# yewzijian/RegTR

Hardware: AMD Instinct MI355X
Metric: point-cloud pairs/sec (3DMatch ~20k pts) (higher is better)
Workload: dtype f32 (f16-pair split, 22-bit operands)

## Files before the change

### regtr_amd/csrc/kpconv.hip

```cpp
#include "common.h"
#include <type_traits>

namespace {

constexpr int KP_PAD = 16;
constexpr int GATHER_WAVES = 4;

__global__ void __launch_bounds__(256) k_rowsum_positive(const float* __restrict__ x, int n, int C, const float2* __restrict__ stats,
                                                         const int* __restrict__ seg_off, int n_seg, float slope,
                                                         float* __restrict__ flag)
{
    const int row = blockIdx.x * (blockDim.x >> 6) + (threadIdx.x >> 6);
    if (row >= n) return;
    const int lane = rg_lane();
    const float2* st = stats ? stats + (size_t)rg_find_segment(seg_off, n_seg, row) * C : nullptr;
    float s = 0.f;
    for (int c = lane; c < C; c += RG_WAVE) {
        float v = x[(size_t)row * C + c];
        if (st) { v = (v - st[c].x) * st[c].y; v = v > 0.f ? v : v * slope; }
        s += v;
    }
    s = rg_wave_sum(s);
    if (lane == 0) flag[row] = s > 0.f ? 1.f : 0.f;
}

struct GatherArgs {
    const float* q_xyz; const float* s_xyz; const int* nbr; const float* x; const float* flag; const float* s_xyzf; const float* kp;
    float* wf; float* num;
    const float2* x_stats; const int* q_seg_off;
    int nq, ns, H, Cin, KP, n_seg, ld_wf;
    float extent, slope;
    int qpw;
};

template <int LQ>
__global__ void __launch_bounds__(GATHER_WAVES * RG_WAVE) k_kpconv_gather(GatherArgs g)
{
    constexpr int QW = RG_WAVE / LQ;
    extern __shared__ __align__(16) float smem[];
    const int wave = threadIdx.x >> 6, lane = rg_lane();
    const int H = g.H;
    const int per_wave = (QW * H * (KP_PAD + 6) + 3) & ~3;
    float* w_s = smem + (size_t)wave * per_wave;
    float* rel_s = w_s + QW * H * KP_PAD;
    int* idx_s = (int*)(rel_s + QW * H * 3);
    float* flg_s = (float*)(idx_s + QW * H);
    float* xs_s = flg_s + QW * H;

    const int q0 = (rg_xcd_block(blockIdx.x, gridDim.x) * GATHER_WAVES + wave) * QW;
    if (q0 >= g.nq) return;

    for (int e = lane; e < QW * H; e += RG_WAVE) {
        const int qi = e / H, h = e - qi * H, q = q0 + qi;
        int idx = g.ns;
        float rx = 1e6f, ry = 1e6f, rz = 1e6f, f = 0.f, x1 = 0.f;
        if (q < g.nq) {
            idx = g.nbr[(size_t)q * H + h];
            float sx = 1e6f, sy = 1e6f, sz = 1e6f;
            if (idx < g.ns) {
                sx = g.s_xyz[3 * (size_t)idx]; sy = g.s_xyz[3 * (size_t)idx + 1]; sz = g.s_xyz[3 * (size_t)idx + 2];
                f = g.flag[idx];
                if (g.Cin == 1) x1 = g.x[idx];
            }
            rx = sx - g.q_xyz[3 * (size_t)q]; ry = sy - g.q_xyz[3 * (size_t)q + 1]; rz = sz - g.q_xyz[3 * (size_t)q + 2];
        }
        idx_s[e] = idx; flg_s[e] = f; xs_s[e] = x1;
        rel_s[3 * e] = rx; rel_s[3 * e + 1] = ry; rel_s[3 * e + 2] = rz;
    }
    __builtin_amdgcn_wave_barrier();

    {
        const int k = lane & (KP_PAD - 1);
        const bool kvalid = k < g.KP;
        const float kx = kvalid ? g.kp[3 * k] : 0.f, ky = kvalid ? g.kp[3 * k + 1] : 0.f, kz = kvalid ? g.kp[3 * k + 2] : 0.f;
        const float inv_extent = 1.0f / g.extent;
        for (int e = lane; e < QW * H * KP_PAD; e += RG_WAVE) {
            const int qh = e >> 4;
            const float dx = rel_s[3 * qh] - kx, dy = rel_s[3 * qh + 1] - ky, dz = rel_s[3 * qh + 2] - kz;
            float d2;
            {
#pragma clang fp contract(off)
                d2 = (dx * dx + dy * dy) + dz * dz;
            }
            float wv = 1.f - __builtin_amdgcn_sqrtf(d2) * inv_extent;
            w_s[e] = (kvalid && wv > 0.f) ? wv : 0.f;
        }
    }
    __builtin_amdgcn_wave_barrier();

    const int qi = lane / LQ, cl = lane % LQ, q = q0 + qi;
    if (q >= g.nq) return;
    const float* wq = w_s + (size_t)qi * H * KP_PAD;
    const int* iq = idx_s + qi * H;
    const int Cin = g.Cin;
    {
        const float2* st = nullptr;
        if (g.x_stats) st = g.x_stats + (size_t)rg_find_segment(g.q_seg_off, g.n_seg, q) * Cin;
        for (int c = cl; c < Cin; c += LQ) {
            float acc[KP_PAD];
#pragma unroll
            for (int k = 0; k < KP_PAD; k++) acc[k] = 0.f;
            float mu = 0.f, rs = 1.f;
            if (st) { mu = st[c].x; rs = st[c].y; }
            for (int h0 = 0; h0 < H; h0 += 8) {
                float xv[8];
#pragma unroll
                for (int u = 0; u < 8; u++) {
                    const int h = h0 + u;
                    const int idx = h < H ? iq[h] : g.ns;
                    xv[u] = idx < g.ns ? g.x[(size_t)idx * Cin + c] : 0.f;
                    if (st && idx < g.ns) { const float t = (xv[u] - mu) * rs; xv[u] = t > 0.f ? t : t * g.slope; }
                }
#pragma unroll
                for (int u = 0; u < 8; u++) {
                    const int h = h0 + u;
                    if (h < H) {
                        const float4* w4 = (const float4*)(wq + h * KP_PAD);
#pragma unroll
                        for (int j = 0; j < KP_PAD / 4; j++) {
                            const float4 wv = w4[j];
                            acc[4 * j + 0] = fmaf(wv.x, xv[u], acc[4 * j + 0]);
                            acc[4 * j + 1] = fmaf(wv.y, xv[u], acc[4 * j + 1]);
                            acc[4 * j + 2] = fmaf(wv.z, xv[u], acc[4 * j + 2]);
                            acc[4 * j + 3] = fmaf(wv.w, xv[u], acc[4 * j + 3]);
                        }
                    }
                }
            }
            float* o = g.wf + (size_t)q * g.KP * Cin + c;
#pragma unroll
            for (int k = 0; k < KP_PAD; k++)
                if (k < g.KP) o[(size_t)k * Cin] = acc[k];
        }
    }
    if (cl == 0) {
        float cnt = 0.f;
        const float* fq = flg_s + qi * H;
        for (int h = 0; h < H; h++) cnt += fq[h];
        g.num[q] = fmaxf(cnt, 1.f);
    }
}


typedef float floatx4 __attribute__((ext_vector_type(4)));
#ifndef RG_MG_QPW
#define RG_MG_QPW 8
#endif
constexpr int MG_QPW = RG_MG_QPW;

template <int V> struct RgVec;
template <> struct RgVec<2> { typedef float2 type; };
template <> struct RgVec<4> { typedef float4 type; };
__device__ __forceinline__ float rg_comp(const float2& v, int i) { return i == 0 ? v.x : v.y; }
__device__ __forceinline__ float rg_comp(const float4& v, int i) { return i == 0 ? v.x : (i == 1 ? v.y : (i == 2 ? v.z : v.w)); }
__device__ __forceinline__ void rg_set(float2& v, int i, float f) { if (i == 0) v.x = f; else v.y = f; }
__device__ __forceinline__ void rg_set(float4& v, int i, float f) { if (i == 0) v.x = f; else if (i == 1) v.y = f; else if (i == 2) v.z = f; else v.w = f; }

__device__ __forceinline__ float rg_row16_sum(float v)
{
    v += __int_as_float(__builtin_amdgcn_update_dpp(0, __float_as_int(v), 0x128, 0xf, 0xf, false));
    v += __int_as_float(__builtin_amdgcn_update_dpp(0, __float_as_int(v), 0x124, 0xf, 0xf, false));
    v += __int_as_float(__builtin_amdgcn_update_dpp(0, __float_as_int(v), 0x122, 0xf, 0xf, false));
    v += __int_as_float(__builtin_amdgcn_update_dpp(0, __float_as_int(v), 0x121, 0xf, 0xf, false));
    return v;
}

typedef unsigned rg_u32x2 __attribute__((ext_vector_type(2)));
typedef unsigned rg_u32x4 __attribute__((ext_vector_type(4)));
constexpr unsigned RG_OOB = 0x80000000u;

__device__ __forceinline__ __amdgpu_buffer_rsrc_t rg_rsrc(const void* p, unsigned bytes)
{
    return __builtin_amdgcn_make_buffer_rsrc(const_cast<void*>(p), 0, bytes, 0x00020000);
}
template <int V> __device__ __forceinline__ typename RgVec<V>::type rg_buf_load(__amdgpu_buffer_rsrc_t r, unsigned off);
template <> __device__ __forceinline__ float2 rg_buf_load<2>(__amdgpu_buffer_rsrc_t r, unsigned off)
{
    const rg_u32x2 v = __builtin_amdgcn_raw_buffer_load_b64(r, off, 0, 0);
    return make_float2(__uint_as_float(v.x), __uint_as_float(v.y));
}
template <> __device__ __forceinline__ float4 rg_buf_load<4>(__amdgpu_buffer_rsrc_t r, unsigned off)
{
    const rg_u32x4 v = __builtin_amdgcn_raw_buffer_load_b128(r, off, 0, 0);
    return make_float4(__uint_as_float(v.x), __uint_as_float(v.y), __uint_as_float(v.z), __uint_as_float(v.w));
}
#ifndef RG_WF_STORE_AUX
#define RG_WF_STORE_AUX 2
#endif
__device__ __forceinline__ void rg_buf_store(__amdgpu_buffer_rsrc_t r, unsigned off, const float2& v)
{
    __builtin_amdgcn_raw_buffer_store_b64(rg_u32x2{__float_as_uint(v.x), __float_as_uint(v.y)}, r, off, 0, RG_WF_STORE_AUX);
}
__device__ __forceinline__ void rg_buf_store(__amdgpu_buffer_rsrc_t r, unsigned off, const float4& v)
{
    __builtin_amdgcn_raw_buffer_store_b128(rg_u32x4{__float_as_uint(v.x), __float_as_uint(v.y), __float_as_uint(v.z), __float_as_uint(v.w)}, r, off, 0, RG_WF_STORE_AUX);
}

typedef float rg_f32x2 __attribute__((ext_vector_type(2)));
#ifndef RG_MG_WAVES_PER_EU
#define RG_MG_WAVES_PER_EU 3
#endif
#ifndef RG_MG_GROUP_STEP
#define RG_MG_GROUP_STEP 1
#endif
#ifndef RG_MG_GROUP_BODIES
#define RG_MG_GROUP_BODIES 6
#endif
template <int J, int V, bool PRE> constexpr int rg_mg_bodies() { return RG_MG_GROUP_BODIES; }
template <> constexpr int rg_mg_bodies<10, 2, false>() { return 1; }
template <int JJ, int JMIN, typename F>
__device__ __forceinline__ void rg_for_group_count(int jn, F&& body)
{
    if constexpr (JJ - RG_MG_GROUP_STEP >= JMIN) {
        if (jn <= JJ - RG_MG_GROUP_STEP) { rg_for_group_count<JJ - RG_MG_GROUP_STEP, JMIN>(jn, body); return; }
    }
    body(std::integral_constant<int, JJ>{});
}
template <int J, int V, bool PRE>
__global__ void __launch_bounds__(GATHER_WAVES * RG_WAVE, RG_MG_WAVES_PER_EU) k_kpconv_gather_mfma(GatherArgs g)
{
    typedef typename RgVec<V>::type vec;
    constexpr int HP = 4 * J;
    __shared__ float4 nb_sh[GATHER_WAVES][HP];
    const int wave = __builtin_amdgcn_readfirstlane(threadIdx.x >> 6), lane = rg_lane();
    const int k = lane & 15, hh = lane >> 4;
    const int H = g.H, Cin = g.Cin, ns = g.ns, nq = g.nq;
    float4* nb_s = nb_sh[wave];
    const bool kvalid = k < g.KP;
    const int kc = kvalid ? k : 0;
    const float kx = kvalid ? g.kp[3 * kc] : 1e30f, ky = g.kp[3 * kc + 1], kz = g.kp[3 * kc + 2];
    const float inv_extent = 1.0f / g.extent;
    const unsigned row_bytes = (unsigned)Cin * 4u;
    const __amdgpu_buffer_rsrc_t x_rs = rg_rsrc(g.x, (unsigned)ns * row_bytes);
    const __amdgpu_buffer_rsrc_t sxyz_rs = rg_rsrc(g.s_xyz, (unsigned)ns * 12u);
    const __amdgpu_buffer_rsrc_t xyzf_rs = rg_rsrc(PRE ? g.s_xyzf : g.s_xyz, PRE ? (unsigned)ns * 16u : 0u);
    const unsigned lane_off = (unsigned)(V * k) * 4u;
    unsigned st_off[4];
#pragma unroll
    for (int r = 0; r < 4; r++) st_off[r] = (4 * hh + r) < g.KP ? (unsigned)(4 * hh + r) * row_bytes + lane_off : RG_OOB;
    const unsigned wf_q_bytes = (unsigned)g.KP * row_bytes;

    const int qpw = g.qpw;
    const int qbase = (rg_xcd_block(blockIdx.x, gridDim.x) * GATHER_WAVES + wave) * qpw;
    if (qbase >= nq) return;
    const int hl = lane < H ? lane : H - 1;
    auto load_idx = [&](int q) -> int {
        const int v = g.nbr[(size_t)(q < nq ? q : nq - 1) * H + hl];
        return (q < nq && lane < H) ? v : ns;
    };
    struct Nb { float rx, ry, rz, f; };
    auto load_nb = [&](int q, int idx) -> Nb {
        const bool real = idx < ns;
        float sx, sy, sz, f = 0.f;
        if (PRE) {
            const rg_u32x4 r = __builtin_amdgcn_raw_buffer_load_b128(xyzf_rs, real ? (unsigned)idx * 16u : RG_OOB, 0, 0);
            sx = __uint_as_float(r.x); sy = __uint_as_float(r.y); sz = __uint_as_float(r.z); f = __uint_as_float(r.w);
        } else {
            const unsigned so = real ? (unsigned)idx * 12u : RG_OOB;
            sx = __uint_as_float(__builtin_amdgcn_raw_buffer_load_b32(sxyz_rs, so, 0, 0));
            sy = __uint_as_float(__builtin_amdgcn_raw_buffer_load_b32(sxyz_rs, so + 4u, 0, 0));
            sz = __uint_as_float(__builtin_amdgcn_raw_buffer_load_b32(sxyz_rs, so + 8u, 0, 0));
        }
        const unsigned qc = (unsigned)(q < nq ? q : nq - 1);
        const float qx = g.q_xyz[3 * qc], qy = g.q_xyz[3 * qc + 1], qz = g.q_xyz[3 * qc + 2];
        Nb n;
        n.rx = (real ? sx : 1e6f) - qx; n.ry = (real ? sy : 1e6f) - qy; n.rz = (real ? sz : 1e6f) - qz; n.f = f;
        return n;
    };
    int idx_cur = load_idx(qbase);
    Nb nb_cur = load_nb(qbase, idx_cur);
    int idx_nxt = load_idx(qbase + 1);
    int seg_cur = 0, seg_end = -1;
#pragma unroll 1
    for (int qq = 0; qq < qpw; qq++) {
        const int q = qbase + qq;
        if (q >= nq) return;
        __builtin_amdgcn_wave_barrier();
        if (lane < HP) {
            const unsigned ro = idx_cur < ns ? (unsigned)idx_cur * row_bytes : RG_OOB;
            nb_s[lane] = make_float4(nb_cur.rx, nb_cur.ry, nb_cur.rz, __uint_as_float(ro));
        }
        __builtin_amdgcn_wave_barrier();
        const float2* st = nullptr;
        if (!PRE && g.x_stats) {
            if (q >= seg_end) {
                seg_cur = rg_find_segment_wave(g.q_seg_off, g.n_seg, q);
                seg_end = g.q_seg_off[seg_cur + 1];
            }
            st = g.x_stats + (size_t)seg_cur * Cin;
        }
        const __amdgpu_buffer_rsrc_t wf_rs = rg_rsrc(g.wf + (size_t)q * g.KP * Cin, wf_q_bytes);
        Nb nb_nxt = nb_cur;
        int idx_nn = ns;
        const float f_cur = nb_cur.f;
        const unsigned long long real = __ballot(idx_cur < ns);
        const int jn = real ? (64 - __builtin_clzll(real) + 3) >> 2 : 0;
        auto body = [&](auto jj) {
            constexpr int JJ = decltype(jj)::value;
            float w[JJ];
            unsigned row[JJ];
#pragma unroll
            for (int j = 0; j < JJ; j++) {
                const float4 nb = nb_s[4 * j + hh];
                const float dx = nb.x - kx, dy = nb.y - ky, dz = nb.z - kz;
                float d2;
                {
#pragma clang fp contract(off)
                    d2 = (dx * dx + dy * dy) + dz * dz;
                }
                w[j] = fmaxf(1.f - __builtin_amdgcn_sqrtf(d2) * inv_extent, 0.f);
                row[j] = __float_as_uint(nb.w) + lane_off;
            }
            float rsum[JJ];
#pragma unroll
            for (int j = 0; j < JJ; j++) rsum[j] = 0.f;
#pragma unroll 1
            for (int c0 = 0; c0 < Cin; c0 += 16 * V) {
                const unsigned c0b = (unsigned)c0 * 4u;
                vec xv[JJ];
#pragma unroll
                for (int j = 0; j < JJ; j++) xv[j] = rg_buf_load<V>(x_rs, row[j] + c0b);
                if (c0 == 0) {
                    nb_nxt = load_nb(q + 1, idx_nxt);
                    idx_nn = load_idx(q + 2);
                }
                if (!PRE && st) {
                    float2 ms[V];
#pragma unroll
                    for (int v = 0; v < V; v += 2) {
                        const float4 t = *(const float4*)(st + c0 + V * k + v);
                        ms[v] = make_float2(t.x, t.y); ms[v + 1] = make_float2(t.z, t.w);
                    }
#pragma unroll
                    for (int j = 0; j < JJ; j++)
#pragma unroll
                        for (int v = 0; v < V; v++) {
                            const float t = (rg_comp(xv[j], v) - ms[v].x) * ms[v].y;
                            rg_set(xv[j], v, fmaxf(t, t * g.slope));
                        }
                }
                if (!PRE)
#pragma unroll
                for (int j = 0; j < JJ; j++) {
                    float s = rg_comp(xv[j], 0);
#pragma unroll
                    for (int v = 1; v < V; v++) s += rg_comp(xv[j], v);
                    rsum[j] += s;
                }
                floatx4 acc[V];
#pragma unroll
                for (int v = 0; v < V; v++) acc[v] = floatx4{0.f, 0.f, 0.f, 0.f};
#pragma unroll
                for (int j = 0; j < JJ; j++)
#pragma unroll
                    for (int v = 0; v < V; v++)
                        acc[v] = __builtin_amdgcn_mfma_f32_16x16x4f32(w[j], rg_comp(xv[j], v), acc[v], 0, 0, 0);
#pragma unroll
                for (int r = 0; r < 4; r++) {
                    vec o;
#pragma unroll
                    for (int v = 0; v < V; v++) rg_set(o, v, acc[v][r]);
                    rg_buf_store(wf_rs, st_off[r] + c0b, o);
                }
            }
            float cnt = 0.f;
            if (PRE) {
                cnt = (float)__builtin_popcountll(__ballot(f_cur > 0.f));
            } else {
#pragma unroll
                for (int j = 0; j < JJ; j++) cnt += (rg_row16_sum(rsum[j]) > 0.f && row[j] < RG_OOB) ? 1.f : 0.f;
                cnt += __shfl_xor(cnt, 16, RG_WAVE);
                cnt += __shfl_xor(cnt, 32, RG_WAVE);
            }
            if (lane == 0) g.num[q] = fmaxf(cnt, 1.f);
        };
        constexpr int JMIN = J - (rg_mg_bodies<J, V, PRE>() - 1) * RG_MG_GROUP_STEP;
        rg_for_group_count<J, (JMIN < 1 ? 1 : JMIN)>(jn, body);
        idx_cur = idx_nxt; nb_cur = nb_nxt; idx_nxt = idx_nn;
    }
}



__device__ __forceinline__ int rg_wave_max_uniform(int v)
{
    v = max(v, __builtin_amdgcn_update_dpp(0, v, 0x128, 0xf, 0xf, false));
    v = max(v, __builtin_amdgcn_update_dpp(0, v, 0x124, 0xf, 0xf, false));
    v = max(v, __builtin_amdgcn_update_dpp(0, v, 0x122, 0xf, 0xf, false));
    v = max(v, __builtin_amdgcn_update_dpp(0, v, 0x121, 0xf, 0xf, false));
    return max(max(__builtin_amdgcn_readlane(v, 0), __builtin_amdgcn_readlane(v, 16)),
               max(__builtin_amdgcn_readlane(v, 32), __builtin_amdgcn_readlane(v, 48)));
}

__global__ void __launch_bounds__(GATHER_WAVES * RG_WAVE) k_kpconv_gather_c1(GatherArgs g)
{
    constexpr int QW = 4;
    extern __shared__ __align__(16) float smem[];
    const int wave = threadIdx.x >> 6, lane = rg_lane();
    const int H = g.H, HP = (H + 1) & ~1, NPAIR = HP >> 1;
    float* pair_s = smem + (size_t)wave * QW * NPAIR * 10;
    const int q0 = (rg_xcd_block(blockIdx.x, gridDim.x) * GATHER_WAVES + wave) * QW;
    if (q0 >= g.nq) return;
    int used = 0;
    for (int e = lane; e < QW * HP; e += RG_WAVE) {
        const int qi = e / HP, h = e - qi * HP, q = q0 + qi;
        float rx = 1e6f, ry = 1e6f, rz = 1e6f, f = 0.f, x1 = 0.f;
        if (q < g.nq && h < H) {
            const int idx = g.nbr[(size_t)q * H + h];
            float sx = 1e6f, sy = 1e6f, sz = 1e6f;
            if (idx < g.ns) {
                used = max(used, h + 1);
                if (g.s_xyzf) {
                    const float4 r = *(const float4*)(g.s_xyzf + 4 * (size_t)idx);
                    sx = r.x; sy = r.y; sz = r.z; x1 = r.w; f = x1 > 0.f ? 1.f : 0.f;
                } else {
                    sx = g.s_xyz[3 * (size_t)idx]; sy = g.s_xyz[3 * (size_t)idx + 1]; sz = g.s_xyz[3 * (size_t)idx + 2];
                    x1 = g.x[idx]; f = g.flag ? g.flag[idx] : (x1 > 0.f ? 1.f : 0.f);
                }
            }
            rx = sx - g.q_xyz[3 * (size_t)q]; ry = sy - g.q_xyz[3 * (size_t)q + 1]; rz = sz - g.q_xyz[3 * (size_t)q + 2];
        }
        float* d = pair_s + (qi * NPAIR + (h >> 1)) * 10 + (h & 1);
        d[0] = rx; d[2] = ry; d[4] = rz; d[6] = x1; d[8] = f;
    }
    __builtin_amdgcn_wave_barrier();
    const int npair = (rg_wave_max_uniform(used) + 1) >> 1;
    const int qi = lane >> 4, k = lane & 15, q = q0 + qi;
    if (q >= g.nq) return;
    const bool kvalid = k < g.KP;
    const float kx = kvalid ? g.kp[3 * k] : 0.f, ky = kvalid ? g.kp[3 * k + 1] : 0.f, kz = kvalid ? g.kp[3 * k + 2] : 0.f;
    const float inv_extent = 1.0f / g.extent;
    const rg_f32x2 ninv{-inv_extent, -inv_extent}, one{1.f, 1.f};
    float acc = 0.f, cnt = 0.f;
    const float* pp = pair_s + qi * NPAIR * 10;
    for (int p = 0; p < npair; p++, pp += 10) {
        const rg_f32x2 dx = *(const rg_f32x2*)(pp) - kx, dy = *(const rg_f32x2*)(pp + 2) - ky, dz = *(const rg_f32x2*)(pp + 4) - kz;
        const rg_f32x2 xv = *(const rg_f32x2*)(pp + 6), fv = *(const rg_f32x2*)(pp + 8);
        rg_f32x2 d2;
        {
#pragma clang fp contract(off)
            d2 = (dx * dx + dy * dy) + dz * dz;
        }
        const rg_f32x2 sq{__builtin_amdgcn_sqrtf(d2.x), __builtin_amdgcn_sqrtf(d2.y)};
        const rg_f32x2 t = __builtin_elementwise_fma(sq, ninv, one);
        acc = fmaf(fmaxf(t.x, 0.f), xv.x, acc);
        acc = fmaf(fmaxf(t.y, 0.f), xv.y, acc);
        cnt += fv.x + fv.y;
    }
    if (k < g.ld_wf) g.wf[(size_t)q * g.ld_wf + k] = kvalid ? acc : 0.f;
    if (k == 0) g.num[q] = fmaxf(cnt, 1.f);
}

template <int NS>
__global__ void __launch_bounds__(GATHER_WAVES * RG_WAVE) k_kpconv_gather_c1p(GatherArgs g)
{
    constexpr int QW = 4;
    extern __shared__ __align__(16) float smem[];
    const int wave = __builtin_amdgcn_readfirstlane(threadIdx.x >> 6), lane = rg_lane();
    const int H = g.H, HP = (H + 1) & ~1, NPAIR = HP >> 1, nq = g.nq, ns = g.ns;
    float* buf_s = smem + (size_t)wave * 2 * QW * NPAIR * 10;
    const int groups = g.qpw;
    const int qbase = (rg_xcd_block(blockIdx.x, gridDim.x) * GATHER_WAVES + wave) * QW * groups;
    if (qbase >= nq) return;
    int e_q[NS], e_h[NS], e_dst[NS];
#pragma unroll
    for (int s = 0; s < NS; s++) {
        const int e = lane + RG_WAVE * s;
        e_q[s] = e / HP; e_h[s] = e - e_q[s] * HP;
        if (e >= QW * HP) { e_q[s] = -1; e_h[s] = 0; }
        e_dst[s] = (e_q[s] * NPAIR + (e_h[s] >> 1)) * 10 + (e_h[s] & 1);
    }
    auto issue_idx = [&](int qg, int (&idx)[NS]) {
#pragma unroll
        for (int s = 0; s < NS; s++) {
            const int q = qg + (e_q[s] < 0 ? 0 : e_q[s]);
            const int v = g.nbr[(size_t)(q < nq ? q : nq - 1) * H + (e_h[s] < H ? e_h[s] : H - 1)];
            idx[s] = (e_q[s] >= 0 && q < nq && e_h[s] < H) ? v : -1;
        }
    };
    struct Rec { float4 r; float qx, qy, qz; };
    auto issue_rec = [&](int qg, const int (&idx)[NS], Rec (&rec)[NS]) {
#pragma unroll
        for (int s = 0; s < NS; s++) {
            const int q = qg + (e_q[s] < 0 ? 0 : e_q[s]);
            const unsigned qc = (unsigned)(q < nq ? q : nq - 1);
            const int ic = idx[s] < 0 ? 0 : (idx[s] < ns ? idx[s] : ns - 1);
            rec[s].r = *(const float4*)(g.s_xyzf + 4 * (size_t)ic);
            rec[s].qx = g.q_xyz[3 * qc]; rec[s].qy = g.q_xyz[3 * qc + 1]; rec[s].qz = g.q_xyz[3 * qc + 2];
        }
    };
    auto stage = [&](float* buf, const int (&idx)[NS], const Rec (&rec)[NS]) -> int {
        int used = 0;
#pragma unroll
        for (int s = 0; s < NS; s++) {
            if (e_q[s] < 0) continue;
            const bool elem = idx[s] >= 0, real = elem && idx[s] < ns;
            used = real ? max(used, e_h[s] + 1) : used;
            const float sx = real ? rec[s].r.x : 1e6f, sy = real ? rec[s].r.y : 1e6f, sz = real ? rec[s].r.z : 1e6f;
            const float x1 = real ? rec[s].r.w : 0.f;
            float* d = buf + e_dst[s];
            d[0] = elem ? sx - rec[s].qx : 1e6f; d[2] = elem ? sy - rec[s].qy : 1e6f; d[4] = elem ? sz - rec[s].qz : 1e6f;
            d[6] = x1; d[8] = x1 > 0.f ? 1.f : 0.f;
        }
        return (rg_wave_max_uniform(used) + 1) >> 1;
    };
    const int qi = lane >> 4, k = lane & 15;
    const bool kvalid = k < g.KP;
    const float kx = kvalid ? g.kp[3 * k] : 0.f, ky = kvalid ? g.kp[3 * k + 1] : 0.f, kz = kvalid ? g.kp[3 * k + 2] : 0.f;
    const float inv_extent = 1.0f / g.extent;
    const rg_f32x2 ninv{-inv_extent, -inv_extent}, one{1.f, 1.f};

    int idx_a[NS], idx_b[NS];
    Rec rec[NS];
    issue_idx(qbase, idx_a);
    issue_rec(qbase, idx_a, rec);
    issue_idx(qbase + QW, idx_b);
    int npair = stage(buf_s, idx_a, rec);
#pragma unroll 1
    for (int gi = 0; gi < groups; gi++) {
        const int qg = qbase + gi * QW;
        if (qg >= nq) return;
        int idx_c[NS];
        issue_rec(qg + QW, idx_b, rec);
        issue_idx(qg + 2 * QW, idx_c);
        __builtin_amdgcn_wave_barrier();
        const int q = qg + qi;
        const float* pp = buf_s + (gi & 1) * QW * NPAIR * 10 + qi * NPAIR * 10;
        float acc = 0.f, cnt = 0.f;
        for (int p = 0; p < npair; p++, pp += 10) {
            const rg_f32x2 dx = *(const rg_f32x2*)(pp) - kx, dy = *(const rg_f32x2*)(pp + 2) - ky, dz = *(const rg_f32x2*)(pp + 4) - kz;
            const rg_f32x2 xv = *(const rg_f32x2*)(pp + 6), fv = *(const rg_f32x2*)(pp + 8);
            rg_f32x2 d2;
            {
#pragma clang fp contract(off)
                d2 = (dx * dx + dy * dy) + dz * dz;
            }
            const rg_f32x2 sq{__builtin_amdgcn_sqrtf(d2.x), __builtin_amdgcn_sqrtf(d2.y)};
            const rg_f32x2 t = __builtin_elementwise_fma(sq, ninv, one);
            acc = fmaf(fmaxf(t.x, 0.f), xv.x, acc);
            acc = fmaf(fmaxf(t.y, 0.f), xv.y, acc);
            cnt += fv.x + fv.y;
        }
        if (q < nq) {
            if (k < g.ld_wf) g.wf[(size_t)q * g.ld_wf + k] = kvalid ? acc : 0.f;
            if (k == 0) g.num[q] = fmaxf(cnt, 1.f);
        }
        __builtin_amdgcn_wave_barrier();
        npair = stage(buf_s + ((gi + 1) & 1) * QW * NPAIR * 10, idx_b, rec);
#pragma unroll
        for (int s = 0; s < NS; s++) idx_b[s] = idx_c[s];
    }
}

template <int QW>
__global__ void __launch_bounds__(256) k_maxpool_gather(const float* __restrict__ x, int ns, int C, const int* __restrict__ nbr,
                                                        int ld_nbr, int nq, int H, float* __restrict__ out)
{
    constexpr int LQ = RG_WAVE / QW;
    const int lane = rg_lane();
    const int q = (rg_xcd_block(blockIdx.x, gridDim.x) * (blockDim.x >> 6) + (threadIdx.x >> 6)) * QW + lane / LQ;
    if (q >= nq) return;
    const int* row = nbr + (size_t)q * ld_nbr;
    for (int c = (lane % LQ) * 4; c < C; c += LQ * 4) {
        float4 m = make_float4(-INFINITY, -INFINITY, -INFINITY, -INFINITY);
        for (int h0 = 0; h0 < H; h0 += 8) {
            float4 v[8];
#pragma unroll
            for (int u = 0; u < 8; u++) {
                const int idx = h0 + u < H ? row[h0 + u] : -1;
                v[u] = m;
                if (idx >= 0) v[u] = idx < ns ? *(const float4*)(x + (size_t)idx * C + c) : make_float4(0.f, 0.f, 0.f, 0.f);
            }
#pragma unroll
            for (int u = 0; u < 8; u++) {
                m.x = fmaxf(m.x, v[u].x); m.y = fmaxf(m.y, v[u].y); m.z = fmaxf(m.z, v[u].z); m.w = fmaxf(m.w, v[u].w);
            }
        }
        *(float4*)(out + (size_t)q * C + c) = m;
    }
}

}

namespace {
constexpr unsigned MP_OOB = 0xfffffff0u;
template <int QW, int HB>
__global__ void __launch_bounds__(256) k_maxpool_gather_buf(const float* __restrict__ x, int ns, int C, const int* __restrict__ nbr,
                                                            int ld_nbr, int nq, int H, float* __restrict__ out)
{
    constexpr int LQ = RG_WAVE / QW;
    const int lane = rg_lane();
    const int q = (rg_xcd_block(blockIdx.x, gridDim.x) * (blockDim.x >> 6) + (threadIdx.x >> 6)) * QW + lane / LQ;
    const int qc = q < nq ? q : nq - 1;
    const int* row = nbr + (size_t)qc * ld_nbr;
    const unsigned row_bytes = (unsigned)C * 4u;
    const __amdgpu_buffer_rsrc_t x_rs = rg_rsrc(x, (unsigned)ns * row_bytes);
    for (int c = (lane % LQ) * 4; c < C; c += LQ * 4) {
        float4 m = make_float4(-INFINITY, -INFINITY, -INFINITY, -INFINITY);
        const unsigned cb = (unsigned)c * 4u;
        for (int h0 = 0; h0 < H; h0 += HB) {
            int idx[HB];
#pragma unroll
            for (int u = 0; u < HB; u++) idx[u] = row[min(h0 + u, H - 1)];
            float4 v[HB];
#pragma unroll
            for (int u = 0; u < HB; u++) v[u] = rg_buf_load<4>(x_rs, (unsigned)idx[u] < (unsigned)ns ? (unsigned)idx[u] * row_bytes + cb : MP_OOB);
#pragma unroll
            for (int u = 0; u < HB; u++) {
                m.x = fmaxf(m.x, v[u].x); m.y = fmaxf(m.y, v[u].y); m.z = fmaxf(m.z, v[u].z); m.w = fmaxf(m.w, v[u].w);
            }
        }
        if (q < nq) *(float4*)(out + (size_t)q * C + c) = m;
    }
}
}

extern "C" {

int regtr_rowsum_positive(const float* x, int n, int C, const float* stats, const int* seg_off, int n_seg, float slope,
                          float* flag, void* stream)
{
    if (!x || !flag || n < 0 || C < 1 || (stats && (!seg_off || n_seg < 1))) return RG_ERR_ARG;
    if (n == 0) return RG_OK;
    k_rowsum_positive<<<rg_cdiv(n, 4), 256, 0, (hipStream_t)stream>>>(x, n, C, (const float2*)stats, seg_off, n_seg, slope,
                                                                       flag);
    RG_RETURN_IF_LAUNCH_FAILED();
    return RG_OK;
}

int regtr_kpconv_gather_computes_flag(int Cin, int H) { return (Cin == 1 || (Cin % 32 == 0 && H <= 64)) ? 1 : 0; }

int regtr_kpconv_gather(const float* q_xyz, int nq, const float* s_xyz, int ns, const int* nbr, int H, const float* x,
                        int Cin, const float* flag, const float* s_xyzf, const float* kernel_points, int KP, float extent,
                        const float* x_stats, const int* q_seg_off, int n_seg, float slope, float* wf, int ld_wf, float* num,
                        void* stream)
{
    if (ld_wf == 0) ld_wf = KP * Cin;
    if (ld_wf != KP * Cin && !(Cin == 1 && ld_wf == KP_PAD)) return RG_ERR_ARG;
    if (!q_xyz || !s_xyz || !nbr || !x || !kernel_points || !wf || !num || nq < 0 || ns < 0 || H < 1 ||
        Cin < 1 || KP < 1 || KP > KP_PAD || !(extent > 0.f) || (x_stats && (!q_seg_off || n_seg < 1)) ||
        (s_xyzf && (x_stats || (uintptr_t)s_xyzf % 16 || (long long)ns * 16 >= (1LL << 31))))
        return RG_ERR_ARG;
    if (!flag && !regtr_kpconv_gather_computes_flag(Cin, H)) return RG_ERR_ARG;
    if (nq == 0) return RG_OK;
    GatherArgs g{q_xyz, s_xyz, nbr, x, flag, s_xyzf, kernel_points, wf, num, (const float2*)x_stats, q_seg_off,
                 nq, ns, H, Cin, KP, n_seg, ld_wf, extent, slope, MG_QPW};
    hipStream_t st = (hipStream_t)stream;
    if (Cin == 1) {
        if (x_stats) return RG_ERR_ARG;
        const int HP1 = (H + 1) & ~1;
        if (s_xyzf && 4 * HP1 <= 4 * RG_WAVE && nq > 0 && ns > 0) {
            int groups = (int)(((long long)nq + 256LL * 8 * GATHER_WAVES * 4 - 1) / (256LL * 8 * GATHER_WAVES * 4));
            groups = groups < 1 ? 1 : (groups > 8 ? 8 : groups);
          if (groups >= 2) {
            g.qpw = groups;
            const size_t ldsp = (size_t)GATHER_WAVES * 2 * 4 * HP1 * 5 * sizeof(float);
            const int gridp = rg_xcd_grid(rg_cdiv(nq, GATHER_WAVES * 4 * groups));
            if (4 * HP1 <= 2 * RG_WAVE) k_kpconv_gather_c1p<2><<<gridp, GATHER_WAVES * RG_WAVE, ldsp, st>>>(g);
            else if (4 * HP1 <= 3 * RG_WAVE) k_kpconv_gather_c1p<3><<<gridp, GATHER_WAVES * RG_WAVE, ldsp, st>>>(g);
            else k_kpconv_gather_c1p<4><<<gridp, GATHER_WAVES * RG_WAVE, ldsp, st>>>(g);
            RG_RETURN_IF_LAUNCH_FAILED();
            return RG_OK;
          }
        }
        const size_t lds1 = (size_t)GATHER_WAVES * 4 * HP1 * 5 * sizeof(float);
        k_kpconv_gather_c1<<<rg_xcd_grid(rg_cdiv(nq, GATHER_WAVES * 4)), GATHER_WAVES * RG_WAVE, lds1, st>>>(g);
        RG_RETURN_IF_LAUNCH_FAILED();
        return RG_OK;
    }
    const bool aligned16 = (((uintptr_t)x | (uintptr_t)wf | (uintptr_t)x_stats) & 15) == 0;
    if (!flag && !(aligned16 && ns > 0 && (long long)ns * Cin < (1LL << 29))) return RG_ERR_ARG;
    if (regtr_kpconv_gather_computes_flag(Cin, H) && aligned16 && ns > 0 && (long long)ns * Cin < (1LL << 29)) {
        int qpw = (int)(((long long)nq + 256 * 12 - 1) / (256 * 12));
        qpw = qpw < 1 ? 1 : (qpw > MG_QPW ? MG_QPW : qpw);
        g.qpw = qpw;
        const int grid_m = rg_xcd_grid(rg_cdiv(nq, GATHER_WAVES * qpw));
        const int J = H <= 40 ? 10 : (H <= 52 ? 13 : 16);
        const bool v4 = Cin % 64 == 0;
        const bool pre = s_xyzf != nullptr;
#define RG_LAUNCH_MG2(JJ, VV) do { if (pre) k_kpconv_gather_mfma<JJ, VV, true><<<grid_m, GATHER_WAVES * RG_WAVE, 0, st>>>(g); \
                                   else k_kpconv_gather_mfma<JJ, VV, false><<<grid_m, GATHER_WAVES * RG_WAVE, 0, st>>>(g); } while (0)
#define RG_LAUNCH_MG(JJ) do { if (v4) RG_LAUNCH_MG2(JJ, 4); else RG_LAUNCH_MG2(JJ, 2); } while (0)
        if (J == 10) RG_LAUNCH_MG(10); else if (J == 13) RG_LAUNCH_MG(13); else RG_LAUNCH_MG(16);
#undef RG_LAUNCH_MG
#undef RG_LAUNCH_MG2
        RG_RETURN_IF_LAUNCH_FAILED();
        return RG_OK;
    }
    const int LQ = Cin <= 16 ? 16 : (Cin <= 32 ? 32 : 64);
    const int QW = RG_WAVE / LQ;
    const size_t lds = (size_t)GATHER_WAVES * ((QW * H * (KP_PAD + 6) + 3) & ~3) * sizeof(float);
    if (lds > 160 * 1024) return RG_ERR_ARG;
    const int grid = rg_xcd_grid(rg_cdiv(nq, GATHER_WAVES * QW));
    if (LQ == 16) k_kpconv_gather<16><<<grid, GATHER_WAVES * RG_WAVE, lds, st>>>(g);
    else if (LQ == 32) k_kpconv_gather<32><<<grid, GATHER_WAVES * RG_WAVE, lds, st>>>(g);
    else k_kpconv_gather<64><<<grid, GATHER_WAVES * RG_WAVE, lds, st>>>(g);
    RG_RETURN_IF_LAUNCH_FAILED();
    return RG_OK;
}


int regtr_maxpool_gather(const float* x, int ns, int C, const int* nbr, int ld_nbr, int nq, int H, float* out, void* stream)
{
    if (!x || !nbr || !out || ns < 0 || nq < 0 || H < 1 || ld_nbr < H || C < 4 || C % 4) return RG_ERR_ARG;
    if (nq == 0) return RG_OK;
    if (ns > 0 && (unsigned long long)ns * C * 4ull < 0xffffff00ull && ((uintptr_t)x % 16) == 0) {
        if (C <= 64) k_maxpool_gather_buf<4, 8><<<rg_xcd_grid(rg_cdiv(nq, 16)), 256, 0, (hipStream_t)stream>>>(x, ns, C, nbr, ld_nbr, nq, H, out);
        else if (C <= 128) k_maxpool_gather_buf<2, 8><<<rg_xcd_grid(rg_cdiv(nq, 8)), 256, 0, (hipStream_t)stream>>>(x, ns, C, nbr, ld_nbr, nq, H, out);
        else k_maxpool_gather_buf<1, 8><<<rg_xcd_grid(rg_cdiv(nq, 4)), 256, 0, (hipStream_t)stream>>>(x, ns, C, nbr, ld_nbr, nq, H, out);
        RG_RETURN_IF_LAUNCH_FAILED();
        return RG_OK;
    }
    if (C <= 64) k_maxpool_gather<4><<<rg_xcd_grid(rg_cdiv(nq, 16)), 256, 0, (hipStream_t)stream>>>(x, ns, C, nbr, ld_nbr, nq, H, out);
    else if (C <= 128) k_maxpool_gather<2><<<rg_xcd_grid(rg_cdiv(nq, 8)), 256, 0, (hipStream_t)stream>>>(x, ns, C, nbr, ld_nbr, nq, H, out);
    else k_maxpool_gather<1><<<rg_xcd_grid(rg_cdiv(nq, 4)), 256, 0, (hipStream_t)stream>>>(x, ns, C, nbr, ld_nbr, nq, H, out);
    RG_RETURN_IF_LAUNCH_FAILED();
    return RG_OK;
}

}
```

Baseline: 2233.

## Count positive neighbors via ballot, shrink LDS pair records, restructure max-pool gather

The Cin=1 gather kernels no longer stage a per-neighbor flag in LDS. The positive-neighbor count is computed with wave ballots and popcounts, which shrinks each pair record from 10 to 8 floats so it can be read as two float4 loads, and the weight clamp uses fmed3. The max-pool gather now loads neighbor indices once per lane and broadcasts them by shuffle. It also finds the last real neighbor so the loop stops early, and seeds the max with 0 when shadow neighbors exist. The max-pool rewrite adds control complexity and changes the shadow-neighbor handling semantics, so correctness depends on padding matching the prior behavior.

```diff
diff --git a/regtr_amd/csrc/kpconv.hip b/regtr_amd/csrc/kpconv.hip
--- a/regtr_amd/csrc/kpconv.hip
+++ b/regtr_amd/csrc/kpconv.hip
@@ -197,6 +197,7 @@
 }
 
 typedef float rg_f32x2 __attribute__((ext_vector_type(2)));
+__device__ __forceinline__ float rg_clamp01(float t) { return __builtin_amdgcn_fmed3f(t, 0.f, 1.f); }
 #ifndef RG_MG_WAVES_PER_EU
 #define RG_MG_WAVES_PER_EU 3
 #endif
@@ -392,20 +393,40 @@
                max(__builtin_amdgcn_readlane(v, 32), __builtin_amdgcn_readlane(v, 48)));
 }
 
+constexpr int C1_PAIR = 8;
+
+__device__ __forceinline__ float rg_c1_pair(const float* pp, float kx, float ky, float kz, float ninv, float acc)
+{
+    const float4 a = *(const float4*)pp, b = *(const float4*)(pp + 4);
+    const rg_f32x2 dx = rg_f32x2{a.x, a.y} - kx, dy = rg_f32x2{a.z, a.w} - ky, dz = rg_f32x2{b.x, b.y} - kz;
+    rg_f32x2 d2;
+    {
+#pragma clang fp contract(off)
+        d2 = (dx * dx + dy * dy) + dz * dz;
+    }
+    const float w0 = rg_clamp01(fmaf(__builtin_amdgcn_sqrtf(d2.x), ninv, 1.f));
+    const float w1 = rg_clamp01(fmaf(__builtin_amdgcn_sqrtf(d2.y), ninv, 1.f));
+    acc = fmaf(w0, b.z, acc);
+    return fmaf(w1, b.w, acc);
+}
+
 __global__ void __launch_bounds__(GATHER_WAVES * RG_WAVE) k_kpconv_gather_c1(GatherArgs g)
 {
     constexpr int QW = 4;
     extern __shared__ __align__(16) float smem[];
     const int wave = threadIdx.x >> 6, lane = rg_lane();
     const int H = g.H, HP = (H + 1) & ~1, NPAIR = HP >> 1;
-    float* pair_s = smem + (size_t)wave * QW * NPAIR * 10;
+    float* pair_s = smem + (size_t)wave * QW * NPAIR * C1_PAIR;
     const int q0 = (rg_xcd_block(blockIdx.x, gridDim.x) * GATHER_WAVES + wave) * QW;
     if (q0 >= g.nq) return;
     int used = 0;
-    for (int e = lane; e < QW * HP; e += RG_WAVE) {
+    int cq[QW] = {0, 0, 0, 0};
+    for (int e0 = 0; e0 < QW * HP; e0 += RG_WAVE) {
+        const int e = e0 + lane;
+        const bool in = e < QW * HP;
         const int qi = e / HP, h = e - qi * HP, q = q0 + qi;
         float rx = 1e6f, ry = 1e6f, rz = 1e6f, f = 0.f, x1 = 0.f;
-        if (q < g.nq && h < H) {
+        if (in && q < g.nq && h < H) {
             const int idx = g.nbr[(size_t)q * H + h];
             float sx = 1e6f, sy = 1e6f, sz = 1e6f;
             if (idx < g.ns) {
@@ -420,8 +441,12 @@
             }
             rx = sx - g.q_xyz[3 * (size_t)q]; ry = sy - g.q_xyz[3 * (size_t)q + 1]; rz = sz - g.q_xyz[3 * (size_t)q + 2];
         }
-        float* d = pair_s + (qi * NPAIR + (h >> 1)) * 10 + (h & 1);
-        d[0] = rx; d[2] = ry; d[4] = rz; d[6] = x1; d[8] = f;
+#pragma unroll
+        for (int Q = 0; Q < QW; Q++) cq[Q] += __builtin_popcountll(__ballot(in && qi == Q && f > 0.f));
+        if (in) {
+            float* d = pair_s + (qi * NPAIR + (h >> 1)) * C1_PAIR + (h & 1);
+            d[0] = rx; d[2] = ry; d[4] = rz; d[6] = x1;
+        }
     }
     __builtin_amdgcn_wave_barrier();
     const int npair = (rg_wave_max_uniform(used) + 1) >> 1;
@@ -429,26 +454,12 @@
     if (q >= g.nq) return;
     const bool kvalid = k < g.KP;
     const float kx = kvalid ? g.kp[3 * k] : 0.f, ky = kvalid ? g.kp[3 * k + 1] : 0.f, kz = kvalid ? g.kp[3 * k + 2] : 0.f;
-    const float inv_extent = 1.0f / g.extent;
-    const rg_f32x2 ninv{-inv_extent, -inv_extent}, one{1.f, 1.f};
-    float acc = 0.f, cnt = 0.f;
-    const float* pp = pair_s + qi * NPAIR * 10;
-    for (int p = 0; p < npair; p++, pp += 10) {
-        const rg_f32x2 dx = *(const rg_f32x2*)(pp) - kx, dy = *(const rg_f32x2*)(pp + 2) - ky, dz = *(const rg_f32x2*)(pp + 4) - kz;
-        const rg_f32x2 xv = *(const rg_f32x2*)(pp + 6), fv = *(const rg_f32x2*)(pp + 8);
-        rg_f32x2 d2;
-        {
-#pragma clang fp contract(off)
-            d2 = (dx * dx + dy * dy) + dz * dz;
-        }
-        const rg_f32x2 sq{__builtin_amdgcn_sqrtf(d2.x), __builtin_amdgcn_sqrtf(d2.y)};
-        const rg_f32x2 t = __builtin_elementwise_fma(sq, ninv, one);
-        acc = fmaf(fmaxf(t.x, 0.f), xv.x, acc);
-        acc = fmaf(fmaxf(t.y, 0.f), xv.y, acc);
-        cnt += fv.x + fv.y;
-    }
+    const float ninv = -(1.0f / g.extent);
+    float acc = 0.f;
+    const float* pp = pair_s + qi * NPAIR * C1_PAIR;
+    for (int p = 0; p < npair; p++, pp += C1_PAIR) acc = rg_c1_pair(pp, kx, ky, kz, ninv, acc);
     if (k < g.ld_wf) g.wf[(size_t)q * g.ld_wf + k] = kvalid ? acc : 0.f;
-    if (k == 0) g.num[q] = fmaxf(cnt, 1.f);
+    if (k == 0) g.num[q] = fmaxf((float)(qi == 0 ? cq[0] : (qi == 1 ? cq[1] : (qi == 2 ? cq[2] : cq[3]))), 1.f);
 }
 
 template <int NS>
@@ -458,17 +469,20 @@
     extern __shared__ __align__(16) float smem[];
     const int wave = __builtin_amdgcn_readfirstlane(threadIdx.x >> 6), lane = rg_lane();
     const int H = g.H, HP = (H + 1) & ~1, NPAIR = HP >> 1, nq = g.nq, ns = g.ns;
-    float* buf_s = smem + (size_t)wave * 2 * QW * NPAIR * 10;
+    float* buf_s = smem + (size_t)wave * 2 * QW * NPAIR * C1_PAIR;
     const int groups = g.qpw;
     const int qbase = (rg_xcd_block(blockIdx.x, gridDim.x) * GATHER_WAVES + wave) * QW * groups;
     if (qbase >= nq) return;
     int e_q[NS], e_h[NS], e_dst[NS];
+    unsigned long long e_of[NS][QW];
 #pragma unroll
     for (int s = 0; s < NS; s++) {
         const int e = lane + RG_WAVE * s;
         e_q[s] = e / HP; e_h[s] = e - e_q[s] * HP;
         if (e >= QW * HP) { e_q[s] = -1; e_h[s] = 0; }
-        e_dst[s] = (e_q[s] * NPAIR + (e_h[s] >> 1)) * 10 + (e_h[s] & 1);
+        e_dst[s] = (e_q[s] * NPAIR + (e_h[s] >> 1)) * C1_PAIR + (e_h[s] & 1);
+#pragma unroll
+        for (int Q = 0; Q < QW; Q++) e_of[s][Q] = __ballot(e_q[s] == Q);
     }
     auto issue_idx = [&](int qg, int (&idx)[NS]) {
 #pragma unroll
@@ -489,8 +503,16 @@
             rec[s].qx = g.q_xyz[3 * qc]; rec[s].qy = g.q_xyz[3 * qc + 1]; rec[s].qz = g.q_xyz[3 * qc + 2];
         }
     };
-    auto stage = [&](float* buf, const int (&idx)[NS], const Rec (&rec)[NS]) -> int {
-        int used = 0;
+    const int qi = lane >> 4, k = lane & 15;
+    auto stage = [&](float* buf, const int (&idx)[NS], const Rec (&rec)[NS], int& cnt) -> int {
+        int used = 0, cq[QW] = {0, 0, 0, 0};
+#pragma unroll
+        for (int s = 0; s < NS; s++) {
+            const unsigned long long pos = __ballot(idx[s] >= 0 && idx[s] < ns && rec[s].r.w > 0.f);
+#pragma unroll
+            for (int Q = 0; Q < QW; Q++) cq[Q] += __builtin_popcountll(pos & e_of[s][Q]);
+        }
+        cnt = qi == 0 ? cq[0] : (qi == 1 ? cq[1] : (qi == 2 ? cq[2] : cq[3]));
 #pragma unroll
         for (int s = 0; s < NS; s++) {
             if (e_q[s] < 0) continue;
@@ -500,22 +522,20 @@
             const float x1 = real ? rec[s].r.w : 0.f;
             float* d = buf + e_dst[s];
             d[0] = elem ? sx - rec[s].qx : 1e6f; d[2] = elem ? sy - rec[s].qy : 1e6f; d[4] = elem ? sz - rec[s].qz : 1e6f;
-            d[6] = x1; d[8] = x1 > 0.f ? 1.f : 0.f;
+            d[6] = x1;
         }
         return (rg_wave_max_uniform(used) + 1) >> 1;
     };
-    const int qi = lane >> 4, k = lane & 15;
     const bool kvalid = k < g.KP;
     const float kx = kvalid ? g.kp[3 * k] : 0.f, ky = kvalid ? g.kp[3 * k + 1] : 0.f, kz = kvalid ? g.kp[3 * k + 2] : 0.f;
-    const float inv_extent = 1.0f / g.extent;
-    const rg_f32x2 ninv{-inv_extent, -inv_extent}, one{1.f, 1.f};
-
-    int idx_a[NS], idx_b[NS];
+    const float ninv = -(1.0f / g.extent);
+
+    int idx_a[NS], idx_b[NS], cnt = 0;
     Rec rec[NS];
     issue_idx(qbase, idx_a);
     issue_rec(qbase, idx_a, rec);
     issue_idx(qbase + QW, idx_b);
-    int npair = stage(buf_s, idx_a, rec);
+    int npair = stage(buf_s, idx_a, rec, cnt);
 #pragma unroll 1
     for (int gi = 0; gi < groups; gi++) {
         const int qg = qbase + gi * QW;
@@ -525,28 +545,15 @@
         issue_idx(qg + 2 * QW, idx_c);
         __builtin_amdgcn_wave_barrier();
         const int q = qg + qi;
-        const float* pp = buf_s + (gi & 1) * QW * NPAIR * 10 + qi * NPAIR * 10;
-        float acc = 0.f, cnt = 0.f;
-        for (int p = 0; p < npair; p++, pp += 10) {
-            const rg_f32x2 dx = *(const rg_f32x2*)(pp) - kx, dy = *(const rg_f32x2*)(pp + 2) - ky, dz = *(const rg_f32x2*)(pp + 4) - kz;
-            const rg_f32x2 xv = *(const rg_f32x2*)(pp + 6), fv = *(const rg_f32x2*)(pp + 8);
-            rg_f32x2 d2;
-            {
-#pragma clang fp contract(off)
-                d2 = (dx * dx + dy * dy) + dz * dz;
-            }
-            const rg_f32x2 sq{__builtin_amdgcn_sqrtf(d2.x), __builtin_amdgcn_sqrtf(d2.y)};
-            const rg_f32x2 t = __builtin_elementwise_fma(sq, ninv, one);
-            acc = fmaf(fmaxf(t.x, 0.f), xv.x, acc);
-            acc = fmaf(fmaxf(t.y, 0.f), xv.y, acc);
-            cnt += fv.x + fv.y;
-        }
+        const float* pp = buf_s + ((gi & 1) * QW + qi) * NPAIR * C1_PAIR;
+        float acc = 0.f;
+        for (int p = 0; p < npair; p++, pp += C1_PAIR) acc = rg_c1_pair(pp, kx, ky, kz, ninv, acc);
         if (q < nq) {
             if (k < g.ld_wf) g.wf[(size_t)q * g.ld_wf + k] = kvalid ? acc : 0.f;
-            if (k == 0) g.num[q] = fmaxf(cnt, 1.f);
+            if (k == 0) g.num[q] = fmaxf((float)cnt, 1.f);
         }
         __builtin_amdgcn_wave_barrier();
-        npair = stage(buf_s + ((gi + 1) & 1) * QW * NPAIR * 10, idx_b, rec);
+        npair = stage(buf_s + ((gi + 1) & 1) * QW * NPAIR * C1_PAIR, idx_b, rec, cnt);
 #pragma unroll
         for (int s = 0; s < NS; s++) idx_b[s] = idx_c[s];
     }
@@ -589,28 +596,57 @@
                                                             int ld_nbr, int nq, int H, float* __restrict__ out)
 {
     constexpr int LQ = RG_WAVE / QW;
-    const int lane = rg_lane();
+    static_assert(LQ % HB == 0 && HB % 2 == 0, "a batch never straddles two index registers");
+    const int lane = rg_lane(), sl = lane % LQ;
     const int q = (rg_xcd_block(blockIdx.x, gridDim.x) * (blockDim.x >> 6) + (threadIdx.x >> 6)) * QW + lane / LQ;
     const int qc = q < nq ? q : nq - 1;
     const int* row = nbr + (size_t)qc * ld_nbr;
     const unsigned row_bytes = (unsigned)C * 4u;
     const __amdgpu_buffer_rsrc_t x_rs = rg_rsrc(x, (unsigned)ns * row_bytes);
-    for (int c = (lane % LQ) * 4; c < C; c += LQ * 4) {
-        float4 m = make_float4(-INFINITY, -INFINITY, -INFINITY, -INFINITY);
+    const int idx0 = row[min(sl, H - 1)];
+    int last = 0;
+    bool sh = false;
+    for (int hc = 0; hc < H; hc += LQ) {
+        const int h = hc + sl;
+        const int id = hc == 0 ? idx0 : row[min(h, H - 1)];
+        const bool real = (unsigned)id < (unsigned)ns;
+        last = (h < H && real) ? h + 1 : last;
+        sh = sh || (h < H && !real);
+    }
+    const int hmax = rg_wave_max_uniform(last);
+    const unsigned long long shm = __ballot(sh);
+    const bool q_sh = ((shm >> (lane - sl)) & (LQ == 64 ? ~0ull : (1ull << (LQ & 63)) - 1ull)) != 0;
+    const float m0 = q_sh ? 0.f : -INFINITY;
+    for (int c0 = 0; c0 < C; c0 += LQ * 4) {
+        const int c = c0 + sl * 4;
+        const bool live = c < C;
+        float4 m = make_float4(m0, m0, m0, m0);
         const unsigned cb = (unsigned)c * 4u;
-        for (int h0 = 0; h0 < H; h0 += HB) {
-            int idx[HB];
-#pragma unroll
-            for (int u = 0; u < HB; u++) idx[u] = row[min(h0 + u, H - 1)];
-            float4 v[HB];
-#pragma unroll
-            for (int u = 0; u < HB; u++) v[u] = rg_buf_load<4>(x_rs, (unsigned)idx[u] < (unsigned)ns ? (unsigned)idx[u] * row_bytes + cb : MP_OOB);
-#pragma unroll
-            for (int u = 0; u < HB; u++) {
+        auto batch = [&](auto nb, int idxr, int j0) {
+            constexpr int NB = decltype(nb)::value;
+            unsigned off[NB];
+#pragma unroll
+            for (int u = 0; u < NB; u++) off[u] = (unsigned)__shfl(idxr, j0 + u, LQ);
+#pragma unroll
+            for (int u = 0; u < NB; u++) off[u] = (int)live & (int)(off[u] < (unsigned)ns) ? off[u] * row_bytes + cb : MP_OOB;
+            float4 v[NB];
+#pragma unroll
+            for (int u = 0; u < NB; u++) v[u] = rg_buf_load<4>(x_rs, off[u]);
+#pragma unroll
+            for (int u = 0; u < NB; u++) {
                 m.x = fmaxf(m.x, v[u].x); m.y = fmaxf(m.y, v[u].y); m.z = fmaxf(m.z, v[u].z); m.w = fmaxf(m.w, v[u].w);
             }
-        }
-        if (q < nq) *(float4*)(out + (size_t)q * C + c) = m;
+        };
+        int idxn = idx0;
+        for (int hc = 0; hc < hmax; hc += LQ) {
+            const int idxr = idxn;
+            idxn = row[min(hc + LQ + sl, H - 1)];
+            const int hend = min(hmax, hc + LQ);
+            int h = hc;
+            for (; hend - h > HB / 2; h += HB) batch(std::integral_constant<int, HB>{}, idxr, h - hc);
+            if (h < hend) batch(std::integral_constant<int, HB / 2>{}, idxr, h - hc);
+        }
+        if (live && q < nq) *(float4*)(out + (size_t)q * C + c) = m;
     }
 }
 }
@@ -654,7 +690,7 @@
             groups = groups < 1 ? 1 : (groups > 8 ? 8 : groups);
           if (groups >= 2) {
             g.qpw = groups;
-            const size_t ldsp = (size_t)GATHER_WAVES * 2 * 4 * HP1 * 5 * sizeof(float);
+            const size_t ldsp = (size_t)GATHER_WAVES * 2 * 4 * (HP1 / 2) * C1_PAIR * sizeof(float);
             const int gridp = rg_xcd_grid(rg_cdiv(nq, GATHER_WAVES * 4 * groups));
             if (4 * HP1 <= 2 * RG_WAVE) k_kpconv_gather_c1p<2><<<gridp, GATHER_WAVES * RG_WAVE, ldsp, st>>>(g);
             else if (4 * HP1 <= 3 * RG_WAVE) k_kpconv_gather_c1p<3><<<gridp, GATHER_WAVES * RG_WAVE, ldsp, st>>>(g);
@@ -663,7 +699,7 @@
             return RG_OK;
           }
         }
-        const size_t lds1 = (size_t)GATHER_WAVES * 4 * HP1 * 5 * sizeof(float);
+        const size_t lds1 = (size_t)GATHER_WAVES * 4 * (HP1 / 2) * C1_PAIR * sizeof(float);
         k_kpconv_gather_c1<<<rg_xcd_grid(rg_cdiv(nq, GATHER_WAVES * 4)), GATHER_WAVES * RG_WAVE, lds1, st>>>(g);
         RG_RETURN_IF_LAUNCH_FAILED();
         return RG_OK;
```

New measurement: 2254 (median of 2 runs). No clear change (+1.0%).
